# sunkafei/coffeedb

Hardware: AMD Instinct MI355X
Metric: sa_build_GiB_per_s (higher is better)
Workload: dtype u64

## Files before the change

### coffeedb_amd/capi.py

```python
import ctypes as C
import os
import subprocess

import numpy as np

_HERE = os.path.dirname(os.path.abspath(__file__))
CSRC = os.path.join(_HERE, "csrc")
LIB_PATH = os.path.join(CSRC, "libcoffeedb_gpu.so")
if os.environ.get("CDB_LIB_PATH"):
    LIB_PATH = os.environ["CDB_LIB_PATH"]
_LIB = None

EXPORTS = [
    "cdb_create", "cdb_destroy", "cdb_last_error", "cdb_add", "cdb_add_bulk", "cdb_build", "cdb_build_view", "cdb_build_views", "cdb_build_device", "cdb_build_resident", "cdb_raw_record_find_string", "cdb_add_raw_record", "cdb_add_raw_dir", "cdb_save", "cdb_load",
    "cdb_query", "cdb_query_or", "cdb_query_ranked", "cdb_query_and", "cdb_query_spans", "cdb_spans_free", "cdb_free", "cdb_query_batch", "cdb_query_batch_offsets", "cdb_hits_free", "cdb_result_free", "cdb_query_batch_device", "cdb_query_batch_offsets_device", "cdb_size", "cdb_bits",
    "cdb_mask", "cdb_sa_width", "cdb_sa_copy", "cdb_set_option", "cdb_get_stat", "cdb_profile_get",
    "cdb_profile_dump", "cdb_profile_reset", "cdb_release_cached_memory", "cdb_cached_memory_bytes", "cdb_set_cache_limit", "cdb_memory_stats", "cdb_memory_reset_peak",
    "cdb_debug_radix_sort", "cdb_debug_verify", "cdb_debug_verify_reference", "cdb_debug_self_check", "cdb_proof_wait", "cdb_layout_rule", "cdb_debug_query_latency",
    "cdb_shards_create", "cdb_shards_destroy", "cdb_shards_last_error", "cdb_shards_add", "cdb_shards_add_bulk", "cdb_shards_set_option",
    "cdb_shards_build", "cdb_shards_query", "cdb_shards_query_batch", "cdb_shards_query_or", "cdb_shards_query_ranked", "cdb_shards_query_spans", "cdb_shards_count", "cdb_shards_get", "cdb_shards_first_doc",
    "cdb_shards_transport", "cdb_shards_build_views", "cdb_shards_query_batch_offsets", "cdb_shards_query_and", "cdb_shards_add_raw_dir", "cdb_shards_save", "cdb_shards_load",
    "cdb_comm_unique_id", "cdb_comm_create", "cdb_comm_create_group", "cdb_comm_destroy", "cdb_comm_last_error", "cdb_comm_merge", "cdb_comm_merge_counts",
    "cdb_comm_world", "cdb_comm_transport", "cdb_reserve", "cdb_reserve_wait",
    "cdb_column_create", "cdb_column_destroy", "cdb_column_last_error", "cdb_column_add_bulk", "cdb_column_build", "cdb_column_query",
    "cdb_column_query_any", "cdb_query_and_columns", "cdb_column_get_stat", "cdb_debug_column_set_option", "cdb_debug_column_profile_dump",
    "cdb_column_cluster", "cdb_cluster", "cdb_clusters_free",
    "cdb_render_rows", "cdb_shards_render_rows", "cdb_rendered_free",
    "cdb_remove", "cdb_column_remove",
    "cdb_append", "cdb_debug_verify_keys",
    "cdb_debug_sort_ws_create", "cdb_debug_sort_ws_destroy", "cdb_debug_radix_sort_ex", "cdb_debug_radix_sort_split",
    "cdb_filter", "cdb_rowset_free", "cdb_rowset_last_error", "cdb_rowset_size", "cdb_rowset_rows", "cdb_rowset_page", "cdb_rowset_cluster",
    "cdb_rowset_cluster_column", "cdb_rowset_get_stat", "cdb_debug_rowset_from_rows", "cdb_debug_rowset_set_option",
    "cdb_debug_rowset_profile_dump",
    "cdb_debug_scan", "cdb_debug_scan_partials", "cdb_debug_stable_ranks",
    "cdb_debug_sweep_records", "cdb_debug_vl_tables",
]


class CdbResult(C.Structure):
    _fields_ = [("npat", C.c_uint64), ("nrows", C.c_uint64), ("nhits", C.c_uint64),
                ("row_ptr", C.POINTER(C.c_uint64)), ("ids", C.POINTER(C.c_int64)), ("counts", C.POINTER(C.c_int64))]


class CdbSpans(C.Structure):
    _fields_ = [("ndocs", C.c_uint64), ("nspans", C.c_uint64), ("ids", C.POINTER(C.c_int64)),
                ("span_ptr", C.POINTER(C.c_uint64)), ("begin", C.POINTER(C.c_uint64)), ("end", C.POINTER(C.c_uint64))]


class CdbHits(C.Structure):
    _fields_ = [("hit_ptr", C.POINTER(C.c_uint64)), ("offsets", C.POINTER(C.c_uint64))]
# ... 1218 lines not shown

def debug_stable_ranks(flags, device=-1):
    lib = load_library()
    lib.cdb_debug_stable_ranks.argtypes = [C.c_int, C.c_void_p, C.c_uint64, C.c_void_p, C.c_void_p, C.POINTER(C.c_uint64)]
    flags = np.ascontiguousarray(flags, dtype=np.uint8)
    n = flags.shape[0]
    before = np.zeros(n, dtype=np.uint64)
    tile_base = np.zeros(max((n + 4095) // 4096, 1), dtype=np.uint64)
    total = C.c_uint64(0)
    rc = lib.cdb_debug_stable_ranks(device, flags.ctypes.data, n, before.ctypes.data, tile_base.ctypes.data, C.byref(total))
    if rc != 0:
        raise ScanError("cdb_debug_stable_ranks", rc)
    return before, tile_base[:(n + 4095) // 4096], total.value


class CdbDebugSweepArgs(C.Structure):
    _fields_ = [("text", C.c_void_p), ("n", C.c_uint64), ("doc_start", C.c_void_p), ("ndocs", C.c_uint64), ("bits", C.c_int),
                ("padded", C.c_int), ("codeslot", C.c_void_p), ("slotmap", C.c_void_p), ("src_col", C.c_void_p),
                ("slot_start", C.c_void_p), ("vl", C.c_int), ("base", C.c_uint32), ("nsym", C.c_int), ("part_m", C.c_uint32),
                ("vl_sym", C.c_void_p), ("vl_dec", C.c_void_p), ("key_bits", C.c_int), ("end_len", C.c_int), ("carry", C.c_int),
                ("carry_shift", C.c_int), ("rec_low_bits", C.c_int), ("aux_bytes", C.c_int), ("g0", C.c_uint32), ("g1", C.c_uint32),
                ("gstart", C.c_uint64), ("gelems", C.c_uint64), ("seg_begin", C.c_void_p), ("seg_end", C.c_void_p),
                ("seg_tile_begin", C.c_void_p), ("lead", C.c_int), ("npass", C.c_int), ("tile_counts", C.c_void_p),
                ("out_k", C.c_void_p), ("out_v", C.c_void_p), ("out_w", C.c_void_p), ("out_hist", C.c_void_p),
                ("out_tile_base", C.c_void_p), ("out_tile_doc", C.c_void_p), ("out_guard_ok", C.POINTER(C.c_int))]


class SweepError(RuntimeError):

    def __init__(self, what, status):
# ... 96 lines not shown
```

### coffeedb_amd/csrc/capi.hip

```cpp
#include <dirent.h>

#include <algorithm>
#include <chrono>
#include <condition_variable>
#include <cstdlib>
#include <cstring>
#include <thread>

#include "../../include/coffeedb_gpu.h"
#include "index_impl.h"

using namespace cdb;

namespace {

static_assert((int)Status::Invalid == CDB_E_INVALID && (int)Status::Device == CDB_E_DEVICE && (int)Status::Internal == CDB_E_INTERNAL,
              "errors.h: Status restates the CDB_E_* codes");

void set_error(Index& ix, const std::string& msg) {
    std::lock_guard<std::mutex> g(ix.err_mu);
    ix.err = msg;
}

template <typename F>
// ... 1570 lines not shown
    else if (!std::strcmp(name, "force_doubling")) ix.force_doubling = value != 0;
    else if (!std::strcmp(name, "initial_passes")) ix.initial_passes = (int)value;
    else if (!std::strcmp(name, "sort_variant")) ix.sort_variant = (int)value;
    else if (!std::strcmp(name, "keyhist3")) ix.keyhist3 = value != 0;
    else if (!std::strcmp(name, "key_symbols")) ix.key_symbols = (int)value;
    else if (!std::strcmp(name, "msd_first")) ix.msd_first = value != 0;
    else if (!std::strcmp(name, "msd_pair")) ix.msd_pair = value != 0;
    else if (!std::strcmp(name, "overlap_paircount")) ix.overlap_paircount = value != 0;
    else if (!std::strcmp(name, "key_directory")) { ix.key_directory = value != 0; ix.h_keydir.clear(); ix.keydir_tried = false; }
    else if (!std::strcmp(name, "fuse_records")) ix.fuse_records = value != 0;
    else if (!std::strcmp(name, "sweep_records")) ix.sweep_records = value != 0;
    else if (!std::strcmp(name, "partial_symbol")) ix.partial_symbol = value != 0;
    else if (!std::strcmp(name, "group_sort")) ix.group_sort = value != 0;
    else if (!std::strcmp(name, "list_rounds")) ix.list_rounds = value != 0;
    else if (!std::strcmp(name, "carried_bits")) ix.carried_bits = value < 0 ? -1 : (value > 6 ? 6 : (int)value);
    else if (!std::strcmp(name, "fuse_pairclass")) ix.fuse_pairclass = value != 0;
    else if (!std::strcmp(name, "group_sort_cap")) ix.group_sort_cap = (int)std::max<int64_t>(1, std::min<int64_t>(value, 1 << 20));
    else if (!std::strcmp(name, "vl_keys")) ix.vl_keys = value < 0 ? 0 : (value > 56 ? 56 : (int)value);
    else if (!std::strcmp(name, "pack_sa")) ix.pack_sa = value != 0;
    else if (!std::strcmp(name, "key_cost_model")) ix.key_cost_model = value != 0;
    else if (!std::strcmp(name, "gen_prebased")) ix.gen_prebased = value != 0;
    else if (!std::strcmp(name, "pack_entries")) ix.pack_entries = value != 0;
    else if (!std::strcmp(name, "segmented_sort")) ix.segmented_sort = value != 0;
    else if (!std::strcmp(name, "fold_root")) ix.fold_root = value != 0;
    else if (!std::strcmp(name, "fold_depth1")) ix.fold_depth1 = value != 0;
    else if (!std::strcmp(name, "flags_in_last_pass")) ix.flags_in_last_pass = value != 0;
    else if (!std::strcmp(name, "search_lanes")) ix.search_lanes = (value == 1 || value == 8) ? (int)value : 0;
    else if (!std::strcmp(name, "digit_bits")) ix.digit_bits = (int)value;
    else if (!std::strcmp(name, "fuse_keygen")) ix.fuse_keygen = value != 0;
    else if (!std::strcmp(name, "force_big_path")) ix.force_big_path = value != 0;
// ... 29 lines not shown
    else {
        set_error(ix, std::string("unknown option: ") + name);
        return CDB_E_INVALID;
    }
    return CDB_OK;
}

int cdb_get_stat(const cdb_index* h, const char* name, double* value) {
    if (!h || !name || !value) return CDB_E_INVALID;
    const BuildStats& b = h->ix.bstats;
    const QueryStats& q = h->ix.qstats;
    struct { const char* n; double v; } tab[] = {
        {"build_ms", b.build_ms}, {"alloc_ms", b.alloc_ms}, {"free_ms", b.free_ms}, {"rounds", (double)b.rounds}, {"ext_rounds", (double)b.ext_rounds},
        {"dbl_rounds", (double)b.dbl_rounds}, {"unresolved_after_initial", (double)b.unresolved_initial},
        {"unresolved_max", (double)b.unresolved_max}, {"sort_passes", (double)b.sort_passes},
        {"sort_passes_skipped", (double)b.sort_passes_skipped}, {"isa_built", (double)b.isa_built}, {"fused_keygen", (double)b.fused_keygen}, {"dense_keys", (double)b.dense_keys}, {"key_layout", (double)b.key_layout}, {"bucketed", (double)b.bucketed}, {"bucket_groups", (double)b.bucket_groups}, {"segmented", (double)b.segmented}, {"fused_records", (double)b.fused_records}, {"sweep_records", (double)b.sweep_records}, {"vl_key_bits", (double)b.vl_key_bits}, {"partial_levels", (double)b.partial_levels}, {"list_rounds", (double)b.list_rounds}, {"pairclass_fused", (double)b.pairclass_fused}, {"group_sorts", (double)b.group_sorts}, {"group_sort_fallbacks", (double)b.group_sort_fallbacks}, {"carried_key_bits", (double)b.carried_key_bits}, {"carried_rounds", (double)b.carried_rounds}, {"unresolved_after_carried", (double)b.unresolved_after_carried}, {"vl_avg_len", b.vl_avg_len}, {"vl_rate", b.vl_rate}, {"vl_est_unresolved", b.vl_est_unresolved}, {"fixed_est_unresolved", b.fixed_est_unresolved}, {"gen_prebased", (double)b.gen_prebased}, {"root_folded", (double)b.root_folded}, {"flags_in_last_pass", (double)b.flags_in_last_pass}, {"msd_first", (double)b.msd_first}, {"bucket_low_digits", (double)b.bucket_low_digits}, {"key_directory_cells", h->ix.h_keydir.empty() ? 0.0 : (double)(h->ix.h_keydir.size() - 1)}, {"group_fallbacks", (double)h->ix.group_fallbacks}, {"dense_key_retries", (double)h->ix.dense_key_retries}, {"self_check_fallbacks", (double)h->ix.self_check_fallbacks}, {"sa_packed", h->ix.sa_packed ? 1.0 : 0.0}, {"sa_bytes_per_entry", h->ix.sa_packed ? 5.0 : (double)h->ix.width}, {"self_check_pairs", (double)h->ix.self_check_pairs}, {"self_check_ms", h->ix.self_check_ms}, {"self_check_coverage", h->ix.size > 1 ? (double)h->ix.self_check_pairs / (double)(h->ix.size - 1) : 0.0},
        {"order_proved", (h->ix.proof.state.load() == 2 || h->ix.proof.state.load() == 3 || (h->ix.self_check == 2 && h->ix.width != 0)) ? 1.0 : 0.0},
        {"proof_state", (double)h->ix.proof.state.load()}, {"proof_ms", h->ix.proof.ms}, {"proof_repair_ms", h->ix.proof.repair_ms},
        {"proof_pairs", (double)h->ix.proof.pairs}, {"proof_bad_pairs", (double)h->ix.proof.found[0]}, {"proof_invalid_entries", (double)h->ix.proof.found[1]}, {"proof_skipped_pairs", (double)h->ix.proof.skipped}, {"proof_mixed_pairs", (double)h->ix.proof.mixed},
        {"proof_runs", (double)h->ix.proof.runs}, {"pool_big_mallocs", (double)DevPool::get().big_mallocs()}, {"premap_ms", h->ix.proof.premap_ms}, {"premap_bytes", (double)h->ix.proof.premap_bytes},
        {"key_symbols", (double)b.key_symbols}, {"symbol_bits", (double)b.symbol_bits},
        {"alphabet", (double)b.alphabet}, {"digit_bits", (double)b.digit_bits}, {"final_depth", (double)b.final_depth}, {"compat_rotations", (double)b.compat_rotations},
        {"compat_depth", (double)b.compat_depth},
        {"host_upload_ms", h->ix.host_upload_ms}, {"host_free_ms", h->ix.host_free_ms},
        {"resident_answers", (double)h->ix.res_answers}, {"launched_answers", (double)h->ix.launched_answers}, {"resident_mode", (double)h->ix.resident_mode},
        {"cluster_table_bytes", h->ix.clu.valid ? (double)(h->ix.clu.bytes() + h->ix.idt.bytes()) : 0.0}, {"cluster_classes", (double)h->ix.clu.nclasses},
        {"cluster_prepare_ms", h->ix.clu.prepare_ms}, {"cluster_ms", h->ix.clu.last_ms}, {"cluster_resorted", h->ix.clu.resorted ? 1.0 : 0.0},
        {"removes", (double)h->ix.rm.calls}, {"remove_compactions", (double)h->ix.rm.compactions}, {"remove_rebuilds", (double)h->ix.rm.rebuilds},
        {"remove_docs", (double)h->ix.rm.docs}, {"remove_bytes", (double)h->ix.rm.bytes}, {"remove_ms", h->ix.rm.last_ms},
        {"appends", (double)h->ix.ap.calls}, {"append_merges", (double)h->ix.ap.merges}, {"append_rebuilds", (double)h->ix.ap.rebuilds},
        {"append_docs", (double)h->ix.ap.docs}, {"append_bytes", (double)h->ix.ap.bytes}, {"append_ms", h->ix.ap.last_ms},
// ... 162 lines not shown
```

### coffeedb_amd/csrc/index_impl.h

```cpp
#pragma once
#include <atomic>
#include <condition_variable>
#include <functional>
#include <mutex>
#include <thread>
#include <string>
#include <vector>

#include "../../include/coffeedb_gpu.h"
#include "common.h"
#include "radix_sort.h"

namespace cdb {

constexpr int TEXT_PAD = 128;

struct BuildStats {
    double build_ms = 0, alloc_ms = 0, free_ms = 0;
    int rounds = 0;
    int ext_rounds = 0;
    int dbl_rounds = 0;
    uint64_t unresolved_initial = 0;
    uint64_t unresolved_max = 0;
    int sort_passes = 0;
// ... 5 lines not shown
    int bucketed = 0;
    int bucket_low_digits = 0;
    int bucket_groups = 0;
    int root_folded = 0;
    int flags_in_last_pass = 0;
    int msd_first = 0;
    int gen_prebased = 0;
    int fused_records = 0;
    int sweep_records = 0;
    int pairclass_fused = 0;
    int list_rounds = 0;
    int group_sorts = 0, group_sort_fallbacks = 0;
    int carried_key_bits = 0;
    int carried_rounds = 0;
    uint64_t unresolved_after_carried = 0;
    int partial_levels = 0;
    int vl_key_bits = 0;
    double vl_avg_len = 0, vl_rate = 0, vl_est_unresolved = 0, fixed_est_unresolved = 0;
    int segmented = 0;
    uint64_t gather_items = 0;
    int key_symbols = 0, symbol_bits = 0, alphabet = 0, digit_bits = 8;
    uint64_t final_depth = 0;
    uint64_t compat_rotations = 0, compat_depth = 0;
};

struct QueryStats {
    double query_ms = 0;
    double upload_ms = 0, device_ms = 0, download_ms = 0;
    uint64_t nhits = 0, nrows = 0;
    uint64_t batches = 0;
// ... 190 lines not shown
    DevBuf q_spec;
    DevBuf q_pat, q_offs, q_left, q_right, q_hoff, q_keys0, q_keys1, q_flags, q_rowptr, q_ids, q_counts, q_hitptr, q_hitoff;

    bool reference_compat = true;
    bool force_doubling = false;
    int initial_passes = 0;
    int key_symbols = 0;
    int sort_variant = 0;
    int search_lanes = 0;
    bool flags_in_last_pass = true;
    bool fold_depth1 = true;
    bool fold_root = true;
    bool segmented_sort = true;
    bool fuse_records = true;
    bool fuse_pairclass = true;
    int carried_bits = -1;
    bool list_rounds = true;
    int group_sort_cap = 4096;
    bool group_sort = true;
    bool partial_symbol = true;
    int vl_keys = 2;
    bool vl_off_once = false;
    bool sweep_records = true;
    bool pack_entries = true;
    bool msd_first = true;
    bool msd_pair = true;
    bool keyhist3 = true;
    int dense_key_retries = 0;
    int group_fallbacks = 0;
    uint64_t bucket_group_limit = 0;
// ... 296 lines not shown
```

### coffeedb_amd/csrc/sa_build.hip

```cpp
#include <algorithm>
#include <chrono>
#include <cmath>
#include <cstdlib>
#include <cstring>

#include "sa_build_phases.h"
#include "records_sweep.h"
#include "vl_code.h"
#include "scan.h"

#ifndef RS_GATHER_ABL
#define RS_GATHER_ABL 0
#endif

namespace cdb {

double now_ms() {
    using namespace std::chrono;
    return duration<double, std::milli>(steady_clock::now().time_since_epoch()).count();
}

namespace {

constexpr int KG_TILE = 2048;
// ... 987 lines not shown
            for (int k = 0; k < nsym2; ++k) {
                const uint32_t byte = k < 8 ? (uint32_t)(lo >> (8 * k)) & 0xFFu : b8;
                const uint64_t sym = (uint64_t)k < rem ? (uint64_t)symmap[byte] : 0ull;
                key2 = (key2 << symbits) | sym;
            }
        } else {
            for (int k = 0; k < nsym2; ++k) {
                const uint64_t sym = (uint64_t)k < rem ? (uint64_t)symmap[p[k]] : 0ull;
                key2 = (key2 << symbits) | sym;
            }
        }
    }
    skey[j] |= key2;
}

constexpr uint32_t FC_TILES_PER_WAVE = 4;
__device__ __forceinline__ void fc_load(const uint8_t* __restrict__ flags, uint64_t n, uint64_t base, uint32_t (&x)[4]) {
    x[0] = x[1] = x[2] = x[3] = 0;
    if (base + 16 <= n) {
        const uint4 w = *reinterpret_cast<const uint4*>(flags + base);
        x[0] = w.x; x[1] = w.y; x[2] = w.z; x[3] = w.w;
    } else if (base < n) {
        for (int k = 0; k < 16 && base + k < n; ++k) x[k >> 2] |= (uint32_t)flags[base + k] << (8 * (k & 3));
    }
}
__device__ __forceinline__ uint32_t fc_count(const uint32_t (&x)[4]) {
    uint32_t cu = 0, ch = 0;
#pragma unroll
    for (int q = 0; q < 4; ++q) {
        const uint32_t u = (x[q] >> 1) & 0x01010101u;
        cu += __popc(u);
        ch += __popc(u & x[q] & 0x01010101u);
    }
    return cu | (ch << 16);
}
__global__ __launch_bounds__(256) void sa_flag_count_kernel(const uint8_t* __restrict__ flags, uint64_t n, uint64_t tiles, U2* __restrict__ partials) {
    static_assert(SC_TILE == 4096, "flag compaction assumes 4096-flag tiles");
    const int lane = threadIdx.x & 63, wave = threadIdx.x >> 6;
    const uint64_t t0 = ((uint64_t)blockIdx.x * 4 + wave) * FC_TILES_PER_WAVE;
#pragma unroll
    for (uint32_t k = 0; k < FC_TILES_PER_WAVE; ++k) {
        const uint64_t tile = t0 + k;
        if (tile >= tiles) break;
        uint32_t v = 0;
#pragma unroll
        for (int c = 0; c < 4; ++c) {
            uint32_t x[4];
            fc_load(flags, n, tile * SC_TILE + (uint64_t)c * 1024 + (uint64_t)lane * 16, x);
            v += fc_count(x);
        }
// ... 1685 lines not shown
        ix.key_base = kp.kbase;
    } else {
        is.sorted_keys.release();
        is.sorted_k32.release();
        is.sorted_low.release();
    }
    ix.bstats.free_ms += now_ms() - ta;
}

struct RefineBuffers {
    DevBuf d_order;
    DevBuf U, skey[2], sval[2], nh, rank, hcov;
    DevBuf d_open;
    DevBuf U2b, lf;
    DevBuf d_gs_state;
};

SlotOrder make_slot_order(Index& ix, const InitialSort& is, const Alphabet& al, DevBuf& d_order) {
    SlotOrder order;
    if (is.folded_roots.empty()) return order;
    const std::vector<Depth1Fold>& depth1 = is.depth1;
    struct Blk { unsigned long long a, len; int code, cls; };
    std::vector<Blk> blks;
    std::vector<int> code_of_root;
    {
        for (int b = 128; b < 256; ++b) if (al.h_map[b]) code_of_root.push_back(al.h_map[b]);
        for (int b = 0; b < 128; ++b) if (al.h_map[b]) code_of_root.push_back(al.h_map[b]);
    }
    for (size_t b = 0; b < is.folded_roots.size(); ++b) {
        const CompatBucket r = is.folded_roots[b];
// ... 41 lines not shown
    DevBuf &d_open = rb.d_open, &U2b = rb.U2b, &lf = rb.lf, &d_gs_state = rb.d_gs_state;
    uint32_t h_acc = 0;
    uint64_t h = is.refine_depth0 ? is.refine_depth0 : (uint64_t)kp.nsym;
    bool isa = false;
    uint64_t cap = 0;
    d_open.alloc(sizeof(uint64_t));
    bool have_list = false;
    uint64_t m_list = 0;
    int list_rs = 0;
    d_gs_state.alloc(2 * sizeof(unsigned long long));
    bool group_sort_on = ix.group_sort;
    const uint32_t carry = is.carry;
    bool carried_pending = carry > 0, list_is_carried = false;
    uint32_t kb_shared = vl_kb1;
    st.carried_rounds = 0;
    for (uint32_t iter = 0;; ++iter) {
        if (iter > 0 && !list_is_carried) {
            uint64_t still = 0;
            CDB_HIP(hipMemcpyAsync(&still, d_open.p, sizeof(still), hipMemcpyDeviceToHost, s));
            CDB_HIP(hipStreamSynchronize(s));
            if (still == 0) break;
        }
        const bool carried = carried_pending;
        carried_pending = false;
        CDB_HIP(hipMemsetAsync(d_open.p, 0, sizeof(uint64_t), s));
        auto flag_tile_sums = [&]() {
            const uint64_t nb = ceil_div(n, SC_TILE);
            ix.scan_partials.ensure(scan_partials_slots(nb) * sizeof(U2));
            int t = ix.prof.begin(s);
            hipLaunchKernelGGL(sa_flag_count_kernel, dim3((unsigned)ceil_div(nb, (uint64_t)(4 * FC_TILES_PER_WAVE))), dim3(256), 0, s,
// ... 3 lines not shown
        bool from_list = have_list && ix.list_rounds;
        have_list = false;
        if (from_list) {
            const uint64_t nb = ceil_div(m_list, SC_TILE);
            ix.scan_partials.ensure(scan_partials_slots(nb) * sizeof(U2));
            int t = ix.prof.begin(s);
            hipLaunchKernelGGL(sa_flag_count_kernel, dim3((unsigned)ceil_div(nb, (uint64_t)(4 * FC_TILES_PER_WAVE))), dim3(256), 0, s,
                               (const uint8_t*)lf.as<uint8_t>(), m_list, nb, ix.scan_partials.as<U2>());
            ix.prof.end(t, "sa_flag_count", m_list, s);
        } else if (!is.tile_sums_ready) {
            flag_tile_sums();
        }
        U2 tot = scan_totals_from_partials<U2>(s, ix.scan_partials, from_list ? m_list : n, OpAdd{}, U2{0, 0});
        is.tile_sums_ready = false;
        uint64_t m = tot.a, G = tot.b;
        if (iter == 0) st.unresolved_initial = st.unresolved_after_carried = m;
        if (list_is_carried) st.unresolved_after_carried = m;
        st.unresolved_max = std::max(st.unresolved_max, m);
        if (m == 0) break;
        if (m >= (1ull << 32) - 4096) throw InternalError("too many unresolved suffixes for one refinement round (internal limit: 2^32)");
        const int gbits = bit_width64(G - 1);
        int nsym2 = std::min((64 - gbits) / symbits, KG_LOOK);
        if (!isa && !carried) {
            const bool use_text = !ix.force_doubling && nsym2 >= 1 &&
                                  ((m <= n / 32 && st.ext_rounds < 4) || (m <= n / 8 && st.ext_rounds < 2));
            if (!use_text) {
                rank.alloc((n + D + 1) * sizeof(R));
                CDB_HIP(hipMemsetAsync(rank.p, 0, (n + D + 1) * sizeof(R), s));
                AllHeadIn ain{flags.as<uint8_t>()};
                (void)scan_totals<uint64_t>(s, ix.scan_partials, ain, n, OpMax{}, (uint64_t)0);
                IsaOut<SAW, R> iout{sa, doc_start, (int)ix.bits, ix.mask, rank.as<R>(), order};
// ... 81 lines not shown
            rs = radix_sort<uint64_t, V>(s, ix.rws, ix.prof, skey[0].as<uint64_t>(), skey[1].as<uint64_t>(),
                                         sval[0].as<V>(), sval[1].as<V>(), m, 0, kbits + gbits, &ss, ix.sort_variant);
            radix_check_error(s, ix.rws);
        }
        hipLaunchKernelGGL((sa_newhead_kernel<I>), dim3((unsigned)ceil_div(m, 256)), dim3(256), 0, s,
                           (const uint64_t*)skey[rs].as<uint64_t>(), (const I*)U.as<I>(),
                           (const uint8_t*)flags.as<uint8_t>(), m, nh.as<uint8_t>());
        const uint64_t hnew = isa ? 2 * h : h + (uint64_t)nsym2;
        {
            int t = ix.prof.begin(s);
            if (carried) {
                hipLaunchKernelGGL((sa_update_kernel<SAW, I, true>), dim3((unsigned)ceil_div(m, 256)), dim3(256), 0, s,
                                   (const V*)sval[rs].as<V>(), (const I*)U.as<I>(), (const uint8_t*)nh.as<uint8_t>(), m,
                                   doc_start, (int)ix.bits, ix.mask, (uint64_t)0, sa, flags.as<uint8_t>(), (unsigned long long*)nullptr,
                                   (const uint8_t*)nullptr, 0u, lf.as<uint8_t>());
                st.carried_rounds++;
                kb_shared = vl_kb1 + carry;
                have_list = true;
                m_list = m;
                list_rs = rs;
            } else if (isa) {
                HeadIn<I> hin{nh.as<uint8_t>(), U.as<I>()};
                (void)scan_totals<uint64_t>(s, ix.scan_partials, hin, m, OpMax{}, (uint64_t)0);
                UpdateOut<SAW, I, R> uo{sval[rs].as<V>(), U.as<I>(), nh.as<uint8_t>(), m, doc_start, (int)ix.bits,
                                      ix.mask, hnew, sa, flags.as<uint8_t>(), rank.as<R>(), d_open.as<unsigned long long>(), order};
                scan_apply<uint64_t>(s, ix.scan_partials, hin, m, OpMax{}, (uint64_t)0, uo);
                st.dbl_rounds++;
            } else {
                hipLaunchKernelGGL((sa_update_kernel<SAW, I>), dim3((unsigned)ceil_div(m, 256)), dim3(256), 0, s,
                                   (const V*)sval[rs].as<V>(), (const I*)U.as<I>(), (const uint8_t*)nh.as<uint8_t>(), m,
                                   doc_start, (int)ix.bits, ix.mask, hnew, sa, flags.as<uint8_t>(), d_open.as<unsigned long long>(),
// ... 227 lines not shown
```

### include/coffeedb_gpu.h

```cpp
#ifndef COFFEEDB_GPU_H
#define COFFEEDB_GPU_H

#include <stddef.h>
#include <stdint.h>

#ifdef __cplusplus
extern "C" {
#endif

#define CDB_OK 0
#define CDB_E_INVALID 1
#define CDB_E_DEVICE 2
#define CDB_E_INTERNAL 3

typedef struct cdb_index cdb_index;

typedef struct cdb_result {
    uint64_t npat;
    uint64_t nrows;
    uint64_t nhits;
    uint64_t* row_ptr;
    int64_t* ids;
    int64_t* counts;
} cdb_result;
// ... 303 lines not shown
    const uint64_t* seg_end;
    const uint32_t* seg_tile_begin;
    int lead, npass;
    const uint32_t* tile_counts;
    uint32_t* out_k;
    uint32_t* out_v;
    void* out_w;
    uint64_t* out_hist;
    uint64_t* out_tile_base;
    uint64_t* out_tile_doc;
    int* out_guard_ok;
} cdb_debug_sweep_args;
int cdb_debug_sweep_records(int device, const cdb_debug_sweep_args* args);
int cdb_debug_vl_tables(const uint64_t* counts, int sigma, const uint8_t* slot_of_code, uint16_t* sym_out, uint16_t* dec_out, int* end_len_out);

int cdb_debug_query_latency(cdb_index* h, const char* blob, const uint64_t* offsets, size_t nkw, int reps, double* us_out);

int cdb_layout_rule(uint64_t ndocs, uint64_t longest, uint64_t* bits, uint64_t* mask, int* width, int* off_bits,
                    char* err, size_t err_cap);

#ifdef __cplusplus
}
#endif
#endif
```

Baseline: 31.03.

## Resolve carried-key groups in place within flag tiles before the general round loop

Adds a kernel that, for builds with carried key bits, scans each 4096-flag tile, compacts unresolved entries into per-wave shared-memory lists, and ranks small groups by their carried key bits directly in place. It rewrites the SA entries and flags and produces the tile partials that the next scan needs. The goal is to avoid the first carried round's global gather, sort and update kernels on large inputs. In exchange it adds a host sync to read back counters, and the in-wave ranking is complex and only handles groups that fit within one 64-entry trip.

```diff
diff --git a/coffeedb_amd/capi.py b/coffeedb_amd/capi.py
--- a/coffeedb_amd/capi.py
+++ b/coffeedb_amd/capi.py
@@ -34,6 +34,7 @@
     "cdb_debug_rowset_profile_dump",
     "cdb_debug_scan", "cdb_debug_scan_partials", "cdb_debug_stable_ranks",
     "cdb_debug_sweep_records", "cdb_debug_vl_tables",
+    "cdb_debug_carried_inplace",
 ]
 
 
@@ -1282,6 +1283,35 @@
     return before, tile_base[:(n + 4095) // 4096], total.value
 
 
+CARRIED_PACKED40, CARRIED_U32, CARRIED_U64 = range(3)
+
+
+class CarriedError(RuntimeError):
+
+    def __init__(self, what, status):
+        super().__init__(f"{what} failed ({status})")
+        self.status = status
+
+
+def debug_carried_inplace(entries, flags, xbits, form=CARRIED_PACKED40, device=-1):
+    lib = load_library()
+    lib.cdb_debug_carried_inplace.argtypes = [C.c_int, C.c_int, C.c_void_p, C.c_void_p, C.c_uint64, C.c_int, C.c_void_p, C.c_void_p,
+                                              C.POINTER(C.c_int)]
+    entries = np.array(entries, dtype=np.uint64)
+    flags = np.array(flags, dtype=np.uint8)
+    n = entries.shape[0]
+    if entries.shape != (n,) or flags.shape != (n,):
+        raise ValueError(f"entries of shape {entries.shape}, flags of shape {flags.shape}")
+    partials = np.zeros(((n + 4095) // 4096, 2), dtype=np.uint64)
+    counts = np.zeros(2, dtype=np.uint64)
+    ok = C.c_int(0)
+    rc = lib.cdb_debug_carried_inplace(device, form, entries.ctypes.data if n else None, flags.ctypes.data if n else None, n, xbits,
+                                       partials.ctypes.data, counts.ctypes.data, C.byref(ok))
+    if rc != 0:
+        raise CarriedError("cdb_debug_carried_inplace", rc)
+    return entries, flags, partials, int(counts[0]), int(counts[1]), bool(ok.value)
+
+
 class CdbDebugSweepArgs(C.Structure):
     _fields_ = [("text", C.c_void_p), ("n", C.c_uint64), ("doc_start", C.c_void_p), ("ndocs", C.c_uint64), ("bits", C.c_int),
                 ("padded", C.c_int), ("codeslot", C.c_void_p), ("slotmap", C.c_void_p), ("src_col", C.c_void_p),
diff --git a/coffeedb_amd/csrc/capi.hip b/coffeedb_amd/csrc/capi.hip
--- a/coffeedb_amd/csrc/capi.hip
+++ b/coffeedb_amd/csrc/capi.hip
@@ -1608,6 +1608,7 @@
     else if (!std::strcmp(name, "group_sort")) ix.group_sort = value != 0;
     else if (!std::strcmp(name, "list_rounds")) ix.list_rounds = value != 0;
     else if (!std::strcmp(name, "carried_bits")) ix.carried_bits = value < 0 ? -1 : (value > 6 ? 6 : (int)value);
+    else if (!std::strcmp(name, "carried_inplace")) ix.carried_inplace = value < 0 ? -1 : (value != 0 ? 1 : 0);
     else if (!std::strcmp(name, "fuse_pairclass")) ix.fuse_pairclass = value != 0;
     else if (!std::strcmp(name, "group_sort_cap")) ix.group_sort_cap = (int)std::max<int64_t>(1, std::min<int64_t>(value, 1 << 20));
     else if (!std::strcmp(name, "vl_keys")) ix.vl_keys = value < 0 ? 0 : (value > 56 ? 56 : (int)value);
@@ -1667,7 +1668,7 @@
         {"build_ms", b.build_ms}, {"alloc_ms", b.alloc_ms}, {"free_ms", b.free_ms}, {"rounds", (double)b.rounds}, {"ext_rounds", (double)b.ext_rounds},
         {"dbl_rounds", (double)b.dbl_rounds}, {"unresolved_after_initial", (double)b.unresolved_initial},
         {"unresolved_max", (double)b.unresolved_max}, {"sort_passes", (double)b.sort_passes},
-        {"sort_passes_skipped", (double)b.sort_passes_skipped}, {"isa_built", (double)b.isa_built}, {"fused_keygen", (double)b.fused_keygen}, {"dense_keys", (double)b.dense_keys}, {"key_layout", (double)b.key_layout}, {"bucketed", (double)b.bucketed}, {"bucket_groups", (double)b.bucket_groups}, {"segmented", (double)b.segmented}, {"fused_records", (double)b.fused_records}, {"sweep_records", (double)b.sweep_records}, {"vl_key_bits", (double)b.vl_key_bits}, {"partial_levels", (double)b.partial_levels}, {"list_rounds", (double)b.list_rounds}, {"pairclass_fused", (double)b.pairclass_fused}, {"group_sorts", (double)b.group_sorts}, {"group_sort_fallbacks", (double)b.group_sort_fallbacks}, {"carried_key_bits", (double)b.carried_key_bits}, {"carried_rounds", (double)b.carried_rounds}, {"unresolved_after_carried", (double)b.unresolved_after_carried}, {"vl_avg_len", b.vl_avg_len}, {"vl_rate", b.vl_rate}, {"vl_est_unresolved", b.vl_est_unresolved}, {"fixed_est_unresolved", b.fixed_est_unresolved}, {"gen_prebased", (double)b.gen_prebased}, {"root_folded", (double)b.root_folded}, {"flags_in_last_pass", (double)b.flags_in_last_pass}, {"msd_first", (double)b.msd_first}, {"bucket_low_digits", (double)b.bucket_low_digits}, {"key_directory_cells", h->ix.h_keydir.empty() ? 0.0 : (double)(h->ix.h_keydir.size() - 1)}, {"group_fallbacks", (double)h->ix.group_fallbacks}, {"dense_key_retries", (double)h->ix.dense_key_retries}, {"self_check_fallbacks", (double)h->ix.self_check_fallbacks}, {"sa_packed", h->ix.sa_packed ? 1.0 : 0.0}, {"sa_bytes_per_entry", h->ix.sa_packed ? 5.0 : (double)h->ix.width}, {"self_check_pairs", (double)h->ix.self_check_pairs}, {"self_check_ms", h->ix.self_check_ms}, {"self_check_coverage", h->ix.size > 1 ? (double)h->ix.self_check_pairs / (double)(h->ix.size - 1) : 0.0},
+        {"sort_passes_skipped", (double)b.sort_passes_skipped}, {"isa_built", (double)b.isa_built}, {"fused_keygen", (double)b.fused_keygen}, {"dense_keys", (double)b.dense_keys}, {"key_layout", (double)b.key_layout}, {"bucketed", (double)b.bucketed}, {"bucket_groups", (double)b.bucket_groups}, {"segmented", (double)b.segmented}, {"fused_records", (double)b.fused_records}, {"sweep_records", (double)b.sweep_records}, {"vl_key_bits", (double)b.vl_key_bits}, {"partial_levels", (double)b.partial_levels}, {"list_rounds", (double)b.list_rounds}, {"pairclass_fused", (double)b.pairclass_fused}, {"group_sorts", (double)b.group_sorts}, {"group_sort_fallbacks", (double)b.group_sort_fallbacks}, {"carried_key_bits", (double)b.carried_key_bits}, {"carried_rounds", (double)b.carried_rounds}, {"unresolved_after_carried", (double)b.unresolved_after_carried}, {"carried_inplace", (double)b.carried_inplace}, {"unresolved_after_inplace", (double)b.unresolved_after_inplace}, {"vl_avg_len", b.vl_avg_len}, {"vl_rate", b.vl_rate}, {"vl_est_unresolved", b.vl_est_unresolved}, {"fixed_est_unresolved", b.fixed_est_unresolved}, {"gen_prebased", (double)b.gen_prebased}, {"root_folded", (double)b.root_folded}, {"flags_in_last_pass", (double)b.flags_in_last_pass}, {"msd_first", (double)b.msd_first}, {"bucket_low_digits", (double)b.bucket_low_digits}, {"key_directory_cells", h->ix.h_keydir.empty() ? 0.0 : (double)(h->ix.h_keydir.size() - 1)}, {"group_fallbacks", (double)h->ix.group_fallbacks}, {"dense_key_retries", (double)h->ix.dense_key_retries}, {"self_check_fallbacks", (double)h->ix.self_check_fallbacks}, {"sa_packed", h->ix.sa_packed ? 1.0 : 0.0}, {"sa_bytes_per_entry", h->ix.sa_packed ? 5.0 : (double)h->ix.width}, {"self_check_pairs", (double)h->ix.self_check_pairs}, {"self_check_ms", h->ix.self_check_ms}, {"self_check_coverage", h->ix.size > 1 ? (double)h->ix.self_check_pairs / (double)(h->ix.size - 1) : 0.0},
         {"order_proved", (h->ix.proof.state.load() == 2 || h->ix.proof.state.load() == 3 || (h->ix.self_check == 2 && h->ix.width != 0)) ? 1.0 : 0.0},
         {"proof_state", (double)h->ix.proof.state.load()}, {"proof_ms", h->ix.proof.ms}, {"proof_repair_ms", h->ix.proof.repair_ms},
         {"proof_pairs", (double)h->ix.proof.pairs}, {"proof_bad_pairs", (double)h->ix.proof.found[0]}, {"proof_invalid_entries", (double)h->ix.proof.found[1]}, {"proof_skipped_pairs", (double)h->ix.proof.skipped}, {"proof_mixed_pairs", (double)h->ix.proof.mixed},
diff --git a/coffeedb_amd/csrc/carried_inplace.h b/coffeedb_amd/csrc/carried_inplace.h
--- /dev/null
+++ b/coffeedb_amd/csrc/carried_inplace.h
@@ -0,0 +1,216 @@
+#pragma once
+#include "common.h"
+#include "scan.h"
+
+namespace cdb {
+
+constexpr uint32_t FC_TILES_PER_WAVE = 4;
+__device__ __forceinline__ void fc_load(const uint8_t* __restrict__ flags, uint64_t n, uint64_t base, uint32_t (&x)[4]) {
+    x[0] = x[1] = x[2] = x[3] = 0;
+    if (base + 16 <= n) {
+        const uint4 w = *reinterpret_cast<const uint4*>(flags + base);
+        x[0] = w.x; x[1] = w.y; x[2] = w.z; x[3] = w.w;
+    } else if (base < n) {
+        for (int k = 0; k < 16 && base + k < n; ++k) x[k >> 2] |= (uint32_t)flags[base + k] << (8 * (k & 3));
+    }
+}
+__device__ __forceinline__ uint32_t fc_count(const uint32_t (&x)[4]) {
+    uint32_t cu = 0, ch = 0;
+#pragma unroll
+    for (int q = 0; q < 4; ++q) {
+        const uint32_t u = (x[q] >> 1) & 0x01010101u;
+        cu += __popc(u);
+        ch += __popc(u & x[q] & 0x01010101u);
+    }
+    return cu | (ch << 16);
+}
+
+constexpr uint32_t CI_GROUP_MAX = 64;
+constexpr uint64_t CARRIED_INPLACE_MIN_N = 1ull << 26;
+constexpr uint32_t CI_LIST = 1024;
+constexpr int CI_TRIPS = 4;
+constexpr uint32_t CI_COUNT_SLOTS = 64;
+constexpr uint64_t CI_MAX_N = 1ull << 37;
+template <typename SAW>
+__global__ __launch_bounds__(256) void sa_carried_inplace_kernel(uint8_t* flags, uint64_t n, uint64_t tiles, int xbits, SAW sa,
+                                                                 U2* __restrict__ partials, unsigned long long* __restrict__ counts) {
+    static_assert(SC_TILE == 4096, "flag sweeps assume 4096-flag tiles");
+    static_assert(CI_GROUP_MAX == 64, "a group is ranked inside one 64-entry trip");
+    static_assert(CI_LIST >= 128 && CI_LIST <= SC_TILE, "a window holds a trip and the entry behind it");
+    using V = typename SAW::val;
+    __shared__ uint16_t s_list[4][CI_LIST];
+    __shared__ uint8_t s_key[4][CI_LIST];
+    __shared__ uint8_t s_src[4][CI_TRIPS][64];
+    const int lane = threadIdx.x & 63, wave = threadIdx.x >> 6;
+    const uint64_t le_mask = lane == 63 ? ~0ull : (2ull << lane) - 1ull;
+    uint16_t* const list = s_list[wave];
+    uint8_t* const key = s_key[wave];
+    const uint32_t kmask = (1u << xbits) - 1u;
+    const uint64_t t0 = ((uint64_t)blockIdx.x * 4 + wave) * FC_TILES_PER_WAVE;
+    uint32_t met = 0, moved_n = 0;
+    for (uint32_t k = 0; k < FC_TILES_PER_WAVE; ++k) {
+        const uint64_t tile = t0 + k;
+        if (tile >= tiles) break;
+        const uint64_t tbase = tile * SC_TILE;
+        uint32_t x[4][4], v[4], incl[4];
+#pragma unroll
+        for (int c = 0; c < 4; ++c) fc_load(flags, n, tbase + (uint64_t)c * 1024 + (uint64_t)lane * 16, x[c]);
+#pragma unroll
+        for (int c = 0; c < 4; ++c) incl[c] = v[c] = fc_count(x[c]);
+#pragma unroll
+        for (int off = 1; off < 64; off <<= 1) {
+#pragma unroll
+            for (int c = 0; c < 4; ++c) {
+                const uint32_t y = __shfl_up(incl[c], off);
+                if (lane >= off) incl[c] += y;
+            }
+        }
+        uint32_t total = 0;
+#pragma unroll
+        for (int c = 0; c < 4; ++c) total += __shfl(incl[c], 63) & 0xFFFFu;
+        if (total == 0) {
+            if (lane == 0) partials[tile] = U2{0, 0};
+            continue;
+        }
+        met += total;
+        uint32_t tail_closed = 1;
+        if (__shfl((x[3][3] >> 25) & 1u, 63) != 0 && tbase + SC_TILE < n) {
+            const uint32_t f = flags[tbase + SC_TILE];
+            tail_closed = (!((f >> 1) & 1u) || (f & 1u)) ? 1u : 0u;
+        }
+        uint32_t left_open = 0, left_heads = 0;
+        for (uint32_t pass_lo = 0; pass_lo < total;) {
+            uint32_t cpre = 0;
+#pragma unroll
+            for (int c = 0; c < 4; ++c) {
+                const uint32_t ctot = __shfl(incl[c], 63);
+                if (v[c] & 0xFFFFu) {
+                    uint32_t slot = ((cpre + incl[c] - v[c]) & 0xFFFFu) - pass_lo;
+                    uint32_t um = 0, hm = 0;
+#pragma unroll
+                    for (int w = 0; w < 4; ++w) {
+                        const uint32_t u = (x[c][w] >> 1) & 0x01010101u;
+                        um |= (((u * 0x01020408u) >> 24) & 0xFu) << (4 * w);
+                        hm |= ((((u & x[c][w]) * 0x01020408u) >> 24) & 0xFu) << (4 * w);
+                    }
+                    const uint32_t off0 = (uint32_t)c * 1024u + (uint32_t)lane * 16u;
+                    while (um) {
+                        const uint32_t q = (uint32_t)__builtin_ctz(um);
+                        um &= um - 1u;
+                        if (slot < CI_LIST) {
+                            const uint32_t word = q < 8u ? (q < 4u ? x[c][0] : x[c][1]) : (q < 12u ? x[c][2] : x[c][3]);
+                            list[slot] = (uint16_t)((off0 + q) | (((hm >> q) & 1u) << 12));
+                            key[slot] = (uint8_t)(((word >> (8u * (q & 3u))) & 0xFFu) >> 2);
+                        }
+                        ++slot;
+                    }
+                }
+                cpre += ctot;
+            }
+            __builtin_amdgcn_fence(__ATOMIC_RELEASE, "wavefront");
+            __builtin_amdgcn_wave_barrier();
+            __builtin_amdgcn_fence(__ATOMIC_ACQUIRE, "wavefront");
+            const uint32_t wend = total - pass_lo < CI_LIST ? total : pass_lo + CI_LIST;
+            uint32_t b0 = pass_lo;
+            auto in_window = [&](uint32_t b) { return b < wend && (b + 64u < total ? b + 64u < wend : total <= wend); };
+            while (in_window(b0)) {
+                uint32_t t_off[CI_TRIPS], t_src[CI_TRIPS], t_nf[CI_TRIPS];
+                bool t_moved[CI_TRIPS], t_wr[CI_TRIPS];
+#pragma unroll
+                for (int u = 0; u < CI_TRIPS; ++u) {
+                    t_off[u] = t_src[u] = t_nf[u] = 0;
+                    t_moved[u] = t_wr[u] = false;
+                    if (!in_window(b0)) continue;
+                    uint8_t* const src = s_src[wave][u];
+                    const uint32_t r0 = b0 - pass_lo;
+                    const bool live = b0 + (uint32_t)lane < total;
+                    const uint32_t e = live ? (uint32_t)list[r0 + lane] : 0u;
+                    const uint32_t kf = live ? (uint32_t)key[r0 + lane] : 0u;
+                    const uint32_t km = kf & kmask;
+                    const bool head = ((e >> 12) & 1u) != 0;
+                    const uint64_t hb = __builtin_amdgcn_ballot_w64(head);
+                    const uint32_t wlen = total - b0 < 64u ? total - b0 : 64u;
+                    const bool more = b0 + 64u < total;
+                    const uint32_t next_bound = more ? ((uint32_t)list[r0 + 64u] >> 12) & 1u : tail_closed;
+                    const uint32_t last_head = hb ? 63u - (uint32_t)__builtin_clzll(hb) : 0u;
+                    const uint32_t whole = next_bound ? wlen : (hb ? last_head : 0u);
+                    const uint32_t adv = (!next_bound && more && hb && last_head > 0u) ? last_head : wlen;
+                    const bool owned = live && (uint32_t)lane < whole && (hb & le_mask) != 0;
+                    uint32_t gs = 0, ge = 0;
+                    if (owned) {
+                        gs = 63u - (uint32_t)__builtin_clzll(hb & le_mask);
+                        const uint64_t above = hb & ~le_mask;
+                        ge = above ? (uint32_t)__builtin_ctzll(above) - 1u : wlen - 1u;
+                    }
+                    uint32_t pos = (uint32_t)lane;
+                    if (owned) {
+                        for (uint32_t p = gs; p <= ge; ++p) {
+                            const uint32_t kp = (uint32_t)key[r0 + p] & kmask;
+                            pos -= (uint32_t)(p < (uint32_t)lane && kp > km);
+                            pos += (uint32_t)(p > (uint32_t)lane && kp < km);
+                        }
+                    }
+                    src[pos] = (uint8_t)lane;
+                    __builtin_amdgcn_fence(__ATOMIC_RELEASE, "wavefront");
+                    __builtin_amdgcn_wave_barrier();
+                    __builtin_amdgcn_fence(__ATOMIC_ACQUIRE, "wavefront");
+                    const uint32_t sl = (uint32_t)src[lane];
+                    const uint32_t skf = live ? (uint32_t)key[r0 + sl] : 0u;
+                    const uint32_t skm = skf & kmask;
+                    const uint32_t pkm = __shfl(skm, lane > 0 ? lane - 1 : 0);
+                    const bool nhead = head || (owned && skm != pkm);
+                    const uint64_t nhb = __builtin_amdgcn_ballot_w64(nhead);
+                    const bool last = (uint32_t)lane == ge || ((nhb >> ((lane + 1) & 63)) & 1ull) != 0;
+                    const bool nopen = owned ? !(nhead && last) : live;
+                    const uint64_t cons = adv >= 64u ? ~0ull : (1ull << adv) - 1ull;
+                    left_open += (uint32_t)__popcll(__builtin_amdgcn_ballot_w64(nopen) & cons);
+                    left_heads += (uint32_t)__popcll(__builtin_amdgcn_ballot_w64(nopen && nhead) & cons);
+                    t_moved[u] = owned && sl != (uint32_t)lane;
+                    moved_n += (uint32_t)__popcll(__builtin_amdgcn_ballot_w64(t_moved[u]));
+                    t_off[u] = e & 0xFFFu;
+                    t_src[u] = live ? (uint32_t)list[r0 + sl] & 0xFFFu : 0u;
+                    t_nf[u] = (nhead ? 1u : 0u) | (nopen ? 2u : 0u) | (skf << 2);
+                    t_wr[u] = owned && t_nf[u] != ((head ? 1u : 0u) | 2u | (kf << 2));
+                    b0 += adv;
+                }
+                V val[CI_TRIPS];
+#pragma unroll
+                for (int u = 0; u < CI_TRIPS; ++u) {
+                    val[u] = 0;
+                    if (t_moved[u]) val[u] = sa.load(tbase + (uint64_t)t_src[u]);
+                }
+                __builtin_amdgcn_fence(__ATOMIC_ACQ_REL, "wavefront");
+#pragma unroll
+                for (int u = 0; u < CI_TRIPS; ++u) {
+                    if (t_moved[u]) sa.store(tbase + (uint64_t)t_off[u], val[u]);
+                    if (t_wr[u]) flags[tbase + (uint64_t)t_off[u]] = (uint8_t)t_nf[u];
+                }
+                __builtin_amdgcn_fence(__ATOMIC_RELEASE, "wavefront");
+                __builtin_amdgcn_wave_barrier();
+            }
+            pass_lo = b0;
+            __builtin_amdgcn_fence(__ATOMIC_RELEASE, "wavefront");
+            __builtin_amdgcn_wave_barrier();
+        }
+        if (lane == 0) partials[tile] = U2{(uint64_t)left_open, (uint64_t)left_heads};
+    }
+    if (lane == 0 && (met | moved_n))
+        atomicAdd(&counts[blockIdx.x % CI_COUNT_SLOTS], (unsigned long long)met | ((unsigned long long)moved_n << 32));
+}
+
+template <typename SAW>
+inline void launch_carried_inplace(hipStream_t s, uint8_t* flags, uint64_t n, int xbits, SAW sa, U2* partials, unsigned long long* counts) {
+    const uint64_t nb = ceil_div(n, (uint64_t)SC_TILE);
+    if (!nb) return;
+    hipLaunchKernelGGL((sa_carried_inplace_kernel<SAW>), dim3((unsigned)ceil_div(nb, (uint64_t)(4 * FC_TILES_PER_WAVE))), dim3(256), 0, s, flags,
+                       n, nb, xbits, sa, partials, counts);
+}
+inline void carried_inplace_totals(const unsigned long long (&w)[CI_COUNT_SLOTS], uint64_t& met, uint64_t& moved) {
+    met = moved = 0;
+    for (unsigned long long c : w) {
+        met += c & 0xFFFFFFFFull;
+        moved += c >> 32;
+    }
+}
+
+}
diff --git a/coffeedb_amd/csrc/debug_carried.hip b/coffeedb_amd/csrc/debug_carried.hip
--- /dev/null
+++ b/coffeedb_amd/csrc/debug_carried.hip
@@ -0,0 +1,139 @@
+#include <cstdio>
+#include <cstring>
+#include <mutex>
+#include <string>
+#include <vector>
+
+#include "../../include/coffeedb_gpu.h"
+#include "index_impl.h"
+#include "scan.h"
+#include "carried_inplace.h"
+
+using namespace cdb;
+
+namespace {
+
+std::mutex g_err_mu;
+std::string g_err;
+
+template <typename F>
+int guarded_hook(const char* who, F&& f) {
+    const int rc = guarded_call(g_err_mu, g_err, std::forward<F>(f));
+    if (rc != CDB_OK) {
+        std::lock_guard<std::mutex> g(g_err_mu);
+        std::fprintf(stderr, "%s: %s\n", who, g_err.c_str());
+    }
+    return rc;
+}
+
+struct CallStream {
+    hipStream_t s = nullptr;
+    explicit CallStream(int device) {
+        if (device >= 0) CDB_HIP(hipSetDevice(device));
+        CDB_HIP(hipStreamCreateWithFlags(&s, hipStreamNonBlocking));
+    }
+    ~CallStream() {
+        if (!s) return;
+        (void)hipStreamSynchronize(s);
+        DevPool::get().retire_stream(s);
+        (void)hipStreamDestroy(s);
+    }
+    CallStream(const CallStream&) = delete;
+    CallStream& operator=(const CallStream&) = delete;
+};
+
+constexpr unsigned char GUARD_BYTE = 0xA5;
+constexpr uint64_t GUARD = 4096;
+
+struct Guarded {
+    DevBuf buf;
+    uint64_t bytes = 0;
+    void alloc(hipStream_t s, uint64_t b) {
+        bytes = b;
+        buf.alloc(b + 2 * GUARD);
+        CDB_HIP(hipMemsetAsync(buf.p, GUARD_BYTE, b + 2 * GUARD, s));
+    }
+    char* data() { return static_cast<char*>(buf.p) + GUARD; }
+    void upload(hipStream_t s, const void* h) {
+        if (bytes) CDB_HIP(hipMemcpyAsync(data(), h, bytes, hipMemcpyHostToDevice, s));
+    }
+    void download(hipStream_t s, void* h) {
+        if (bytes) CDB_HIP(hipMemcpyAsync(h, data(), bytes, hipMemcpyDeviceToHost, s));
+    }
+    bool guards_intact(hipStream_t s) {
+        std::vector<unsigned char> g(2 * GUARD);
+        CDB_HIP(hipMemcpyAsync(g.data(), buf.p, GUARD, hipMemcpyDeviceToHost, s));
+        CDB_HIP(hipMemcpyAsync(g.data() + GUARD, data() + bytes, GUARD, hipMemcpyDeviceToHost, s));
+        CDB_HIP(hipStreamSynchronize(s));
+        bool ok = true;
+        for (unsigned char b : g) ok &= b == GUARD_BYTE;
+        return ok;
+    }
+};
+
+}
+
+extern "C" {
+
+int cdb_debug_carried_inplace(int device, int form, uint64_t* entries_inout, uint8_t* flags_inout, uint64_t n, int xbits,
+                              uint64_t* out_partials, uint64_t* out_counts, int* out_guard_ok) {
+    if (out_guard_ok) *out_guard_ok = 0;
+    if (form < CDB_DEBUG_CARRIED_PACKED40 || form > CDB_DEBUG_CARRIED_U64 || n == 0 || n >= (1ull << 31) || xbits < 1 || xbits > 6 ||
+        !entries_inout || !flags_inout || !out_partials || !out_counts)
+        return CDB_E_INVALID;
+    return guarded_hook("cdb_debug_carried_inplace", [&] {
+        CallStream cs(device);
+        hipStream_t s = cs.s;
+        StreamScope sscope(s);
+        const uint64_t nb = ceil_div(n, (uint64_t)SC_TILE);
+        Guarded d_flags, d_lo, d_hi, d_part, d_cnt;
+        d_flags.alloc(s, n);
+        d_flags.upload(s, flags_inout);
+        d_part.alloc(s, scan_partials_slots(nb) * sizeof(U2));
+        d_cnt.alloc(s, CI_COUNT_SLOTS * sizeof(unsigned long long));
+        CDB_HIP(hipMemsetAsync(d_cnt.data(), 0, CI_COUNT_SLOTS * sizeof(unsigned long long), s));
+        std::vector<uint32_t> lo;
+        std::vector<uint8_t> hi;
+        if (form == CDB_DEBUG_CARRIED_U64) {
+            d_lo.alloc(s, n * 8);
+            d_lo.upload(s, entries_inout);
+        } else {
+            lo.resize(n);
+            for (uint64_t i = 0; i < n; ++i) lo[i] = (uint32_t)entries_inout[i];
+            d_lo.alloc(s, n * 4);
+            d_lo.upload(s, lo.data());
+            if (form == CDB_DEBUG_CARRIED_PACKED40) {
+                hi.resize(n);
+                for (uint64_t i = 0; i < n; ++i) hi[i] = (uint8_t)(entries_inout[i] >> 32);
+                d_hi.alloc(s, n);
+                d_hi.upload(s, hi.data());
+            }
+        }
+        uint8_t* const fl = reinterpret_cast<uint8_t*>(d_flags.data());
+        U2* const part = reinterpret_cast<U2*>(d_part.data());
+        unsigned long long* const cnt = reinterpret_cast<unsigned long long*>(d_cnt.data());
+        if (form == CDB_DEBUG_CARRIED_PACKED40)
+            launch_carried_inplace(s, fl, n, xbits, Sa40RW{reinterpret_cast<uint32_t*>(d_lo.data()), reinterpret_cast<uint8_t*>(d_hi.data())}, part, cnt);
+        else if (form == CDB_DEBUG_CARRIED_U32)
+            launch_carried_inplace(s, fl, n, xbits, SaRW<uint32_t>{reinterpret_cast<uint32_t*>(d_lo.data())}, part, cnt);
+        else
+            launch_carried_inplace(s, fl, n, xbits, SaRW<uint64_t>{reinterpret_cast<uint64_t*>(d_lo.data())}, part, cnt);
+        CDB_HIP(hipGetLastError());
+        d_flags.download(s, flags_inout);
+        if (form == CDB_DEBUG_CARRIED_U64) d_lo.download(s, entries_inout);
+        else d_lo.download(s, lo.data());
+        if (form == CDB_DEBUG_CARRIED_PACKED40) d_hi.download(s, hi.data());
+        CDB_HIP(hipMemcpyAsync(out_partials, part, nb * sizeof(U2), hipMemcpyDeviceToHost, s));
+        unsigned long long words[CI_COUNT_SLOTS] = {};
+        CDB_HIP(hipMemcpyAsync(words, cnt, sizeof(words), hipMemcpyDeviceToHost, s));
+        CDB_HIP(hipStreamSynchronize(s));
+        carried_inplace_totals(words, out_counts[0], out_counts[1]);
+        if (form != CDB_DEBUG_CARRIED_U64)
+            for (uint64_t i = 0; i < n; ++i) entries_inout[i] = (uint64_t)lo[i] | (form == CDB_DEBUG_CARRIED_PACKED40 ? (uint64_t)hi[i] << 32 : 0ull);
+        bool ok = d_flags.guards_intact(s) && d_lo.guards_intact(s) && d_part.guards_intact(s) && d_cnt.guards_intact(s);
+        if (form == CDB_DEBUG_CARRIED_PACKED40) ok = ok && d_hi.guards_intact(s);
+        if (out_guard_ok) *out_guard_ok = ok ? 1 : 0;
+    });
+}
+
+}
diff --git a/coffeedb_amd/csrc/index_impl.h b/coffeedb_amd/csrc/index_impl.h
--- a/coffeedb_amd/csrc/index_impl.h
+++ b/coffeedb_amd/csrc/index_impl.h
@@ -43,6 +43,8 @@
     int carried_key_bits = 0;
     int carried_rounds = 0;
     uint64_t unresolved_after_carried = 0;
+    int carried_inplace = 0;
+    uint64_t unresolved_after_inplace = 0;
     int partial_levels = 0;
     int vl_key_bits = 0;
     double vl_avg_len = 0, vl_rate = 0, vl_est_unresolved = 0, fixed_est_unresolved = 0;
@@ -263,6 +265,7 @@
     bool segmented_sort = true;
     bool fuse_records = true;
     bool fuse_pairclass = true;
+    int carried_inplace = -1;
     int carried_bits = -1;
     bool list_rounds = true;
     int group_sort_cap = 4096;
diff --git a/coffeedb_amd/csrc/sa_build.hip b/coffeedb_amd/csrc/sa_build.hip
--- a/coffeedb_amd/csrc/sa_build.hip
+++ b/coffeedb_amd/csrc/sa_build.hip
@@ -8,6 +8,7 @@
 #include "records_sweep.h"
 #include "vl_code.h"
 #include "scan.h"
+#include "carried_inplace.h"
 
 #ifndef RS_GATHER_ABL
 #define RS_GATHER_ABL 0
@@ -1025,26 +1026,6 @@
     skey[j] |= key2;
 }
 
-constexpr uint32_t FC_TILES_PER_WAVE = 4;
-__device__ __forceinline__ void fc_load(const uint8_t* __restrict__ flags, uint64_t n, uint64_t base, uint32_t (&x)[4]) {
-    x[0] = x[1] = x[2] = x[3] = 0;
-    if (base + 16 <= n) {
-        const uint4 w = *reinterpret_cast<const uint4*>(flags + base);
-        x[0] = w.x; x[1] = w.y; x[2] = w.z; x[3] = w.w;
-    } else if (base < n) {
-        for (int k = 0; k < 16 && base + k < n; ++k) x[k >> 2] |= (uint32_t)flags[base + k] << (8 * (k & 3));
-    }
-}
-__device__ __forceinline__ uint32_t fc_count(const uint32_t (&x)[4]) {
-    uint32_t cu = 0, ch = 0;
-#pragma unroll
-    for (int q = 0; q < 4; ++q) {
-        const uint32_t u = (x[q] >> 1) & 0x01010101u;
-        cu += __popc(u);
-        ch += __popc(u & x[q] & 0x01010101u);
-    }
-    return cu | (ch << 16);
-}
 __global__ __launch_bounds__(256) void sa_flag_count_kernel(const uint8_t* __restrict__ flags, uint64_t n, uint64_t tiles, U2* __restrict__ partials) {
     static_assert(SC_TILE == 4096, "flag compaction assumes 4096-flag tiles");
     const int lane = threadIdx.x & 63, wave = threadIdx.x >> 6;
@@ -2760,6 +2741,7 @@
     DevBuf d_open;
     DevBuf U2b, lf;
     DevBuf d_gs_state;
+    DevBuf d_inplace;
 };
 
 SlotOrder make_slot_order(Index& ix, const InitialSort& is, const Alphabet& al, DevBuf& d_order) {
@@ -2831,6 +2813,26 @@
     bool carried_pending = carry > 0, list_is_carried = false;
     uint32_t kb_shared = vl_kb1;
     st.carried_rounds = 0;
+    const bool inplace = carry > 0 && n > 0 && n < CI_MAX_N && (ix.carried_inplace < 0 ? n >= CARRIED_INPLACE_MIN_N : ix.carried_inplace != 0);
+    uint64_t met_inplace = 0;
+    st.carried_inplace = 0;
+    if (inplace) {
+        const uint64_t nb = ceil_div(n, SC_TILE);
+        ix.scan_partials.ensure(scan_partials_slots(nb) * sizeof(U2));
+        rb.d_inplace.alloc(CI_COUNT_SLOTS * sizeof(unsigned long long));
+        CDB_HIP(hipMemsetAsync(rb.d_inplace.p, 0, CI_COUNT_SLOTS * sizeof(unsigned long long), s));
+        int t = ix.prof.begin(s);
+        launch_carried_inplace(s, flags.as<uint8_t>(), n, (int)carry, sa, ix.scan_partials.as<U2>(), rb.d_inplace.as<unsigned long long>());
+        ix.prof.end(t, "sa_carried_inplace", n, s);
+        unsigned long long cnt[CI_COUNT_SLOTS] = {};
+        CDB_HIP(hipMemcpyAsync(cnt, rb.d_inplace.p, sizeof(cnt), hipMemcpyDeviceToHost, s));
+        CDB_HIP(hipStreamSynchronize(s));
+        uint64_t moved_inplace = 0;
+        carried_inplace_totals(cnt, met_inplace, moved_inplace);
+        if (t >= 0) ix.prof.pending[t].bytes = n + moved_inplace * 2 * (std::is_same<SAW, Sa40RW>::value ? 5 : sizeof(V));
+        is.tile_sums_ready = true;
+        st.carried_inplace = 1;
+    }
     for (uint32_t iter = 0;; ++iter) {
         if (iter > 0 && !list_is_carried) {
             uint64_t still = 0;
@@ -2864,7 +2866,12 @@
         U2 tot = scan_totals_from_partials<U2>(s, ix.scan_partials, from_list ? m_list : n, OpAdd{}, U2{0, 0});
         is.tile_sums_ready = false;
         uint64_t m = tot.a, G = tot.b;
-        if (iter == 0) st.unresolved_initial = st.unresolved_after_carried = m;
+        if (iter == 0) {
+            st.unresolved_initial = inplace ? met_inplace : m;
+            st.unresolved_after_inplace = st.unresolved_after_carried = m;
+            if (inplace && met_inplace > 0) st.carried_rounds = 1;
+            st.unresolved_max = std::max(st.unresolved_max, st.unresolved_initial);
+        }
         if (list_is_carried) st.unresolved_after_carried = m;
         st.unresolved_max = std::max(st.unresolved_max, m);
         if (m == 0) break;
@@ -2976,7 +2983,7 @@
                                    (const V*)sval[rs].as<V>(), (const I*)U.as<I>(), (const uint8_t*)nh.as<uint8_t>(), m,
                                    doc_start, (int)ix.bits, ix.mask, (uint64_t)0, sa, flags.as<uint8_t>(), (unsigned long long*)nullptr,
                                    (const uint8_t*)nullptr, 0u, lf.as<uint8_t>());
-                st.carried_rounds++;
+                st.carried_rounds = 1;
                 kb_shared = vl_kb1 + carry;
                 have_list = true;
                 m_list = m;
diff --git a/include/coffeedb_gpu.h b/include/coffeedb_gpu.h
--- a/include/coffeedb_gpu.h
+++ b/include/coffeedb_gpu.h
@@ -341,6 +341,12 @@
 int cdb_debug_sweep_records(int device, const cdb_debug_sweep_args* args);
 int cdb_debug_vl_tables(const uint64_t* counts, int sigma, const uint8_t* slot_of_code, uint16_t* sym_out, uint16_t* dec_out, int* end_len_out);
 
+#define CDB_DEBUG_CARRIED_PACKED40 0
+#define CDB_DEBUG_CARRIED_U32 1
+#define CDB_DEBUG_CARRIED_U64 2
+int cdb_debug_carried_inplace(int device, int form, uint64_t* entries_inout, uint8_t* flags_inout, uint64_t n, int xbits,
+                              uint64_t* out_partials, uint64_t* out_counts, int* out_guard_ok);
+
 int cdb_debug_query_latency(cdb_index* h, const char* blob, const uint64_t* offsets, size_t nkw, int reps, double* us_out);
 
 int cdb_layout_rule(uint64_t ndocs, uint64_t longest, uint64_t* bits, uint64_t* mask, int* width, int* off_bits,
```

Result: faster. 31.97 (median of 6 runs) (+3.0%).
